# monkey0head/RePlay_cql

Measured on NVIDIA B200. Metric: CQL updates/sec (batch 1024), higher is better.
Workload: dtype f32 (f16x3: tensor-core fp16 hi/lo 3-term split with exact power-of-two row scales, fp32 accumulate, 1e-4 parity-gated)

## Files before the change

### replay_cql_b200/csrc/capi.cu

```cuda
#include <cstring>
#include <cstdio>
#include <algorithm>
#include "engine.cuh"
#include "update.cuh"
#include "score.cuh"
#include "tc_selftest.cuh"
#include "score_tc.cuh"
#include "score_tc_h.cuh"
#include "topk_staged.cuh"
#include "metrics.cuh"
#include "dp_peer.cuh"
#include "mma_bench.cuh"

using namespace cql;

struct cql_handle {
  Handle h;
  cudaGraphExec_t graph_exec = nullptr;
  cudaStream_t graph_stream = nullptr;
  int64_t graph_launches = 0;
  cudaGraphExec_t batch_graph[2] = {nullptr, nullptr};
  cudaStream_t batch_graph_stream[2] = {nullptr, nullptr};
  int64_t batch_graph_launches[2] = {0, 0};
  void* sbuf[8] = {nullptr, nullptr, nullptr, nullptr, nullptr, nullptr, nullptr, nullptr};
// ... 19 lines not shown
};

static thread_local std::string g_create_error;

int64_t mdp_build_on_device(Handle& h, const int32_t* user_h, const int32_t* item_h, const int64_t* ts_h, const double* rel_h,
                            const double* noise_h, int64_t n, int top_k, float noise_scale, float* obs_out, float* act_out,
                            float* rew_out, float* term_out, int64_t* order_out);

namespace {

void* scratch(cql_handle* ch, int slot, size_t bytes) {
  if (bytes > ch->sbuf_bytes[slot]) {
    if (ch->sbuf[slot]) CQL_CUDA(cudaFree(ch->sbuf[slot]));
    ch->sbuf[slot] = nullptr;
    ch->sbuf_bytes[slot] = 0;
    const size_t cap = bytes + bytes / 4 + 256;
    CQL_CUDA(cudaMalloc(&ch->sbuf[slot], cap));
    ch->sbuf_bytes[slot] = cap;
  }
  return ch->sbuf[slot];
}

void set_kernel_attrs() {
  CQL_CUDA(cudaFuncSetAttribute(mlp_fwd_kernel<2, 2>, cudaFuncAttributeMaxDynamicSharedMemorySize, FWD_SMEM));
  CQL_CUDA(cudaFuncSetAttribute(mlp_fwd_kernel<3, 1>, cudaFuncAttributeMaxDynamicSharedMemorySize, FWD_SMEM));
  CQL_CUDA(cudaFuncSetAttribute(mlp_bwd1_kernel<3, 1, true, false>, cudaFuncAttributeMaxDynamicSharedMemorySize, BWD1_SMEM));
  CQL_CUDA(cudaFuncSetAttribute(mlp_bwd1_kernel<3, 1, false, true>, cudaFuncAttributeMaxDynamicSharedMemorySize, BWD1_SMEM));
  CQL_CUDA(cudaFuncSetAttribute(mlp_bwd1_kernel<2, 2, true, false>, cudaFuncAttributeMaxDynamicSharedMemorySize, BWD1_SMEM));
  CQL_CUDA(cudaFuncSetAttribute(mlp_bwd2_kernel<3, 1>, cudaFuncAttributeMaxDynamicSharedMemorySize, BWD2_SMEM));
  CQL_CUDA(cudaFuncSetAttribute(mlp_bwd2_kernel<2, 2>, cudaFuncAttributeMaxDynamicSharedMemorySize, BWD2_SMEM));
  CQL_CUDA(cudaFuncSetAttribute(k_score_topk, cudaFuncAttributeMaxDynamicSharedMemorySize, score_smem(CQL_MAX_TOPK)));
  CQL_CUDA(cudaFuncSetAttribute(k_score_pairs, cudaFuncAttributeMaxDynamicSharedMemorySize, FWD_SMEM));
  CQL_CUDA(cudaFuncSetAttribute(k_topk_filter_staged, cudaFuncAttributeMaxDynamicSharedMemorySize, (int)TKS_SMEM));
  CQL_CUDA(cudaFuncSetAttribute(tc::tc_fwd_kernel<true, 2, 2>, cudaFuncAttributeMaxDynamicSharedMemorySize, (int)tc::FwdSmem<true, tc::FWD_NPW>::BYTES));
  CQL_CUDA(cudaFuncSetAttribute(tc::tc_fwd_kernel<true, 3, 1>, cudaFuncAttributeMaxDynamicSharedMemorySize, (int)tc::FwdSmem<true, tc::FWD_NPW>::BYTES));
  CQL_CUDA(cudaFuncSetAttribute(tc::tc_fwd_kernel<false, 2, 2>, cudaFuncAttributeMaxDynamicSharedMemorySize, (int)tc::FwdSmem<false, tc::FWD_NPW>::BYTES));
  CQL_CUDA(cudaFuncSetAttribute(tc::tc_fwd_kernel<false, 3, 1>, cudaFuncAttributeMaxDynamicSharedMemorySize, (int)tc::FwdSmem<false, tc::FWD_NPW>::BYTES));
  CQL_CUDA(cudaFuncSetAttribute(tc::tc_score_kernel, cudaFuncAttributeMaxDynamicSharedMemorySize, (int)tc::ScoreSmem::bytes(CQL_MAX_TOPK)));
  CQL_CUDA(cudaFuncSetAttribute(tc::tc_score_h_kernel, cudaFuncAttributeMaxDynamicSharedMemorySize, (int)tc::ScoreSmemH::bytes(CQL_MAX_TOPK)));
  CQL_CUDA(cudaFuncSetAttribute(tc::tc_bwd2_h_kernel<3, 1>, cudaFuncAttributeMaxDynamicSharedMemorySize, (int)tc::B2HCfg::BYTES));
  CQL_CUDA(cudaFuncSetAttribute(tc::tc_bwd2_h_kernel<2, 2>, cudaFuncAttributeMaxDynamicSharedMemorySize, (int)tc::B2HCfg::BYTES));
  CQL_CUDA(cudaFuncSetAttribute(tc::tc_bwd2_h2_kernel<3, 1>, cudaFuncAttributeMaxDynamicSharedMemorySize, (int)tc::B2PCfg::BYTES));
  CQL_CUDA(cudaFuncSetAttribute(tc::tc_bwd2_h2_kernel<2, 2>, cudaFuncAttributeMaxDynamicSharedMemorySize, (int)tc::B2PCfg::BYTES));
  CQL_CUDA(cudaFuncSetAttribute(tc::tc_bwd1_h_kernel<3, 1, true, false>, cudaFuncAttributeMaxDynamicSharedMemorySize, (int)tc::HCfg::SMEM_BYTES));
  CQL_CUDA(cudaFuncSetAttribute(tc::tc_bwd1_h_kernel<3, 1, false, true>, cudaFuncAttributeMaxDynamicSharedMemorySize, (int)tc::HCfg::SMEM_BYTES));
  CQL_CUDA(cudaFuncSetAttribute(tc::tc_bwd1_h_kernel<2, 2, true, false>, cudaFuncAttributeMaxDynamicSharedMemorySize, (int)tc::HCfg::SMEM_BYTES));
  CQL_CUDA(cudaFuncSetAttribute(tc::tc_fwd_h_kernel<2, 2>, cudaFuncAttributeMaxDynamicSharedMemorySize, (int)tc::HCfg::SMEM_BYTES));
  CQL_CUDA(cudaFuncSetAttribute(tc::tc_fwd_h_kernel<3, 1>, cudaFuncAttributeMaxDynamicSharedMemorySize, (int)tc::HCfg::SMEM_BYTES));
  CQL_CUDA(cudaFuncSetAttribute((tc::tc_fwd_h_kernel<3, 1, tc::HCfgS>), cudaFuncAttributeMaxDynamicSharedMemorySize, (int)tc::HCfgS::SMEM_BYTES));
  CQL_CUDA(cudaFuncSetAttribute((tc::tc_fwd_h_kernel<2, 2, tc::HCfgS>), cudaFuncAttributeMaxDynamicSharedMemorySize, (int)tc::HCfgS::SMEM_BYTES));
  CQL_CUDA(cudaFuncSetAttribute((tc::tc_bwd1_h_kernel<3, 1, true, false, tc::HCfgS>), cudaFuncAttributeMaxDynamicSharedMemorySize, (int)tc::HCfgS::SMEM_BYTES));
  CQL_CUDA(cudaFuncSetAttribute((tc::tc_bwd1_h_kernel<3, 1, false, true, tc::HCfgS>), cudaFuncAttributeMaxDynamicSharedMemorySize, (int)tc::HCfgS::SMEM_BYTES));
  CQL_CUDA(cudaFuncSetAttribute((tc::tc_bwd1_h_kernel<2, 2, true, false, tc::HCfgS>), cudaFuncAttributeMaxDynamicSharedMemorySize, (int)tc::HCfgS::SMEM_BYTES));
  CQL_CUDA(cudaFuncSetAttribute(tc::tc_fwd_h2_kernel<3, 1>, cudaFuncAttributeMaxDynamicSharedMemorySize, (int)tc::H2Cfg::SMEM_BYTES));
  CQL_CUDA(cudaFuncSetAttribute(tc::tc_fwd_h2_kernel<2, 2>, cudaFuncAttributeMaxDynamicSharedMemorySize, (int)tc::H2Cfg::SMEM_BYTES));
  CQL_CUDA(cudaFuncSetAttribute(tc::tc_bwd1_h2_kernel<3, 1, true, false>, cudaFuncAttributeMaxDynamicSharedMemorySize, (int)tc::H2B1Cfg::SMEM_BYTES));
  CQL_CUDA(cudaFuncSetAttribute(tc::tc_bwd1_h2_kernel<3, 1, false, true>, cudaFuncAttributeMaxDynamicSharedMemorySize, (int)tc::H2B1Cfg::SMEM_BYTES));
  CQL_CUDA(cudaFuncSetAttribute(tc::tc_bwd1_h2_kernel<2, 2, true, false>, cudaFuncAttributeMaxDynamicSharedMemorySize, (int)tc::H2B1Cfg::SMEM_BYTES));
  CQL_CUDA(cudaFuncSetAttribute(tc::tc_fwd_ts_kernel<2, 2>, cudaFuncAttributeMaxDynamicSharedMemorySize, (int)tc::TsCfg::SMEM_BYTES));
  CQL_CUDA(cudaFuncSetAttribute(tc::tc_fwd_ts_kernel<3, 1>, cudaFuncAttributeMaxDynamicSharedMemorySize, (int)tc::TsCfg::SMEM_BYTES));
  CQL_CUDA(cudaFuncSetAttribute(tc::tc_bwd1_ts_kernel<3, 1, true, false>, cudaFuncAttributeMaxDynamicSharedMemorySize, (int)tc::TsCfg::SMEM_BYTES));
  CQL_CUDA(cudaFuncSetAttribute(tc::tc_bwd1_ts_kernel<3, 1, false, true>, cudaFuncAttributeMaxDynamicSharedMemorySize, (int)tc::TsCfg::SMEM_BYTES));
  CQL_CUDA(cudaFuncSetAttribute(tc::tc_bwd1_ts_kernel<2, 2, true, false>, cudaFuncAttributeMaxDynamicSharedMemorySize, (int)tc::TsCfg::SMEM_BYTES));
  const int f1 = (int)tc::FwdSmem<true, tc::BWD1_NPW>::BYTES, f0 = (int)tc::FwdSmem<false, tc::BWD1_NPW>::BYTES;
  CQL_CUDA(cudaFuncSetAttribute(tc::tc_bwd1_kernel<true, 3, 1, true, false>, cudaFuncAttributeMaxDynamicSharedMemorySize, f1));
  CQL_CUDA(cudaFuncSetAttribute(tc::tc_bwd1_kernel<true, 3, 1, false, true>, cudaFuncAttributeMaxDynamicSharedMemorySize, f1));
  CQL_CUDA(cudaFuncSetAttribute(tc::tc_bwd1_kernel<true, 2, 2, true, false>, cudaFuncAttributeMaxDynamicSharedMemorySize, f1));
  CQL_CUDA(cudaFuncSetAttribute(tc::tc_bwd1_kernel<false, 3, 1, true, false>, cudaFuncAttributeMaxDynamicSharedMemorySize, f0));
  CQL_CUDA(cudaFuncSetAttribute(tc::tc_bwd1_kernel<false, 3, 1, false, true>, cudaFuncAttributeMaxDynamicSharedMemorySize, f0));
  CQL_CUDA(cudaFuncSetAttribute(tc::tc_bwd1_kernel<false, 2, 2, true, false>, cudaFuncAttributeMaxDynamicSharedMemorySize, f0));
  CQL_CUDA(cudaFuncSetAttribute(tc::tc_bwd2_kernel<true, 3, 1>, cudaFuncAttributeMaxDynamicSharedMemorySize, (int)tc::B2Cfg<true>::BYTES));
  CQL_CUDA(cudaFuncSetAttribute(tc::tc_bwd2_kernel<true, 2, 2>, cudaFuncAttributeMaxDynamicSharedMemorySize, (int)tc::B2Cfg<true>::BYTES));
  CQL_CUDA(cudaFuncSetAttribute(tc::tc_bwd2_kernel<false, 3, 1>, cudaFuncAttributeMaxDynamicSharedMemorySize, (int)tc::B2Cfg<false>::BYTES));
  CQL_CUDA(cudaFuncSetAttribute(tc::tc_bwd2_kernel<false, 2, 2>, cudaFuncAttributeMaxDynamicSharedMemorySize, (int)tc::B2Cfg<false>::BYTES));
}

void create_impl(const cql_config* cfg, cql_handle* ch) {
  Handle& h = ch->h;
  CQL_REQUIRE(cfg != nullptr, "cql_create: cfg is NULL");
  CQL_REQUIRE(cfg->struct_size == (int32_t)sizeof(cql_config), "cql_create: cql_config size mismatch (ABI)");
  CQL_REQUIRE(cfg->batch_size >= 1 && cfg->batch_size <= (1 << 20), "cql_create: batch_size out of range");
  CQL_REQUIRE(cfg->n_critics >= 1 && cfg->n_critics <= CQL_MAX_CRITICS, "cql_create: n_critics must be 1..4");
  CQL_REQUIRE(cfg->n_action_samples >= 1 && cfg->n_action_samples <= 10, "cql_create: n_action_samples must be 1..10");
  CQL_REQUIRE(cfg->precision == CQL_PREC_FP32 || cfg->precision == CQL_PREC_TF32X3 || cfg->precision == CQL_PREC_BF16 ||
                  cfg->precision == CQL_PREC_F16X3,
              "cql_create: bad precision");
  CQL_REQUIRE(cfg->squash == CQL_SQUASH_EPS || cfg->squash == CQL_SQUASH_SOFTPLUS, "cql_create: bad squash");
  CQL_REQUIRE(cfg->world_size >= 1 && cfg->rank >= 0 && cfg->rank < cfg->world_size, "cql_create: bad rank/world_size");
  int ndev = 0;
  cudaError_t e = cudaGetDeviceCount(&ndev);
  if (e != cudaSuccess || ndev == 0)
    throw Error{std::string("cql_create: no CUDA device available (") + cudaGetErrorString(e) +
                "); this library has no CPU fallback"};
  CQL_REQUIRE(cfg->device >= 0 && cfg->device < ndev, "cql_create: device ordinal out of range");
  CQL_CUDA(cudaSetDevice(cfg->device));
  cudaDeviceProp prop{};
  CQL_CUDA(cudaGetDeviceProperties(&prop, cfg->device));
  CQL_REQUIRE(prop.major >= 10, "cql_create: built for sm_100a (B200); found an older GPU");
  h.cfg = *cfg;
  h.num_sms = prop.multiProcessorCount;
  h.B = cfg->batch_size; h.n = cfg->n_action_samples; h.C = cfg->n_critics;
  const int B = h.B, n = h.n, C = h.C, n3 = 3 * n;
  h.rsA = n3; h.rsC = n3 + 1;
  CQL_CUDA(cudaStreamCreateWithFlags(&h.own_stream, cudaStreamNonBlocking));
  CQL_CUDA(cudaStreamCreateWithFlags(&h.side_stream, cudaStreamNonBlocking));
  CQL_CUDA(cudaEventCreateWithFlags(&h.ev_fork, cudaEventDisableTiming));
// ... 952 lines not shown
```

### replay_cql_b200/csrc/update.cuh

```cuda
#pragma once
#include <algorithm>
#include <utility>
#include <cstdlib>
#include "engine.cuh"
#include "mlp_tc.cuh"
#include "mlp_tc_ts.cuh"
#include <type_traits>
#include "mlp_tc_bwd1.cuh"
#include "mlp_tc_bwd2.cuh"
#include "mlp_tc_h.cuh"
#include "mlp_tc_h2.cuh"
#include "adam_pack.cuh"

namespace cql {

__host__ __device__ inline uint32_t mix32(uint32_t x) {
  x ^= x >> 16; x *= 0x7feb352du; x ^= x >> 15; x *= 0x846ca68bu; x ^= x >> 16;
  return x;
}
__host__ __device__ inline uint64_t feistel_perm(uint64_t x, uint64_t n, uint64_t key) {
  int bits = 2;
  while (bits < 62 && (1ull << bits) < n) bits += 2;
  const int hb = bits / 2;
  const uint64_t mask = (1ull << hb) - 1;
// ... 417 lines not shown
    __shared__ float gsh[2];
    if (threadIdx.x == 0) dp_wait_scalars(dp, g_t, g_a, gsh[0], gsh[1]);
    __syncthreads();
    g_t = gsh[0];
    g_a = gsh[1];
  }
  if (k.temp_lr > 0.f) lt = adam_scalar(lt, g_t, mt, vt, k.temp_lr, k, *si);
  if (k.alpha_lr > 0.f) la = adam_scalar(la, g_a, ma, va, k.alpha_lr, k, *si);
  const float alpha = fminf(fmaxf(expf(la), 0.f), 1e6f);
  const float inv = 1.f / ((float)k.C * (float)k.B);
  const float coef = alpha * k.cw * inv;
  const int64_t i = (int64_t)blockIdx.x * blockDim.x + threadIdx.x;
  const int rsC = 3 * k.n + 1;
  if (i < (int64_t)k.C * k.B * rsC) {
    const int j = (int)(i % rsC);
    dQ[i] = j < rsC - 1 ? coef * dQ[i] : 2.f * pairv[i / rsC].err / (float)k.B - coef;
  }
  if (i == 0) {
    if (k.temp_lr > 0.f) { scalars[0] = lt; sc_m[0] = mt; sc_v[0] = vt; }
    if (k.alpha_lr > 0.f) { scalars[1] = la; sc_m[1] = ma; sc_v[1] = va; }
    sums[3] = coef;
    metrics[1] = expf(lt);
    metrics[3] = expf(la);
    const float td = sums[0] / (float)k.B;
    const float cons = alpha * (k.cw * (sums[1] * inv - sums[2] * inv) - k.thr);
    metrics[4] = td + cons;
    metrics[6] = td;
  }
  if (dp.world > 1) dp_consume_done(dp, 0, gridDim.x);
}

__global__ void __launch_bounds__(1024) k_actor_dq(const QSrc srcP, const float4* __restrict__ perb,
                                                   const float* __restrict__ scalars, int B, int C,
                                                   float* __restrict__ dQP, float* __restrict__ metrics) {
  tc::grid_dep_wait();
 
  __shared__ float red[32];
  const float T = expf(scalars[0]);
  float s = 0.f;
  for (int b = threadIdx.x; b < B; b += 1024) {
    int arg = 0;
    float qm = q_at(srcP, 0, b);
    for (int c = 1; c < C; ++c) {
      const float q = q_at(srcP, c, b);
      if (q < qm) { qm = q; arg = c; }
    }
    for (int c = 0; c < C; ++c) dQP[(int64_t)c * B + b] = c == arg ? -1.f / (float)B : 0.f;
    s += T * perb[b].y - qm;
  }
  s = block_sum<1024>(s, red);
  if (threadIdx.x == 0) metrics[5] = s / (float)B;
}

__global__ void k_actor_dout(const float* __restrict__ outA, const float* __restrict__ noise_actor,
                             const float4* __restrict__ dXP, const float* __restrict__ scalars, int B, int n_parts,
                             int squash, float* __restrict__ dOutA, const QSrc srcP, const float4* __restrict__ perb,
                             int C, float* __restrict__ part, unsigned int* __restrict__ ticket, float* __restrict__ metrics) {
  tc::grid_dep_wait();
 
  const int b = blockIdx.x * blockDim.x + threadIdx.x;
  if (srcP.q != nullptr) {
    float v = 0.f;
    if (b < B) {
      float qm = q_at(srcP, 0, b);
      for (int c = 1; c < C; ++c) qm = fminf(qm, q_at(srcP, c, b));
      v = expf(scalars[0]) * perb[b].y - qm;
    }
    v = warp_sum(v);
    if ((threadIdx.x & 31) == 0) part[b >> 5] = v;
    __shared__ bool last;
    __threadfence();
    __syncthreads();
    if (threadIdx.x == 0) {
      const unsigned int t = atomicAdd(ticket, 1u);
      last = t == gridDim.x - 1;
      if (last) *ticket = 0;
    }
    __syncthreads();
    if (last && threadIdx.x < 32) {
      __threadfence();
      const int n_w = (gridDim.x * blockDim.x) >> 5;
      float s = 0.f;
      for (int i = threadIdx.x; i < n_w; i += 32) s += part[i];
      s = warp_sum(s);
      if (threadIdx.x == 0) metrics[5] = s / (float)B;
    }
  }
  if (b >= B) return;
  float da = 0.f;
  for (int c = 0; c < n_parts; ++c) da += dXP[(int64_t)c * B + b].z;
  const float mu = outA[2 * b], ls_raw = outA[2 * b + 1], ls = clamp_ls(ls_raw);
  const float eps = noise_actor[b];
  const Sample s = policy_sample(mu, ls, eps, squash);
  const float w = __fdiv_rn(expf(scalars[0]), (float)B);
  const float one_m_a2 = __fsub_rn(1.f, __fmul_rn(s.a, s.a));
  const float dt_std = __fmul_rn(w, __fdiv_rn(s.t, s.std_));
  float g_tanh;
  if (squash == CQL_SQUASH_EPS) {
    const float g_a = __fadd_rn(da, __fmul_rn(w, __fdiv_rn(__fmul_rn(2.f, s.a), __fadd_rn(one_m_a2, 1e-6f))));
    g_tanh = __fmul_rn(g_a, one_m_a2);
  } else {
    const float sig = __fdiv_rn(1.f, __fadd_rn(1.f, expf(__fmul_rn(2.f, s.raw))));
    g_tanh = __fadd_rn(__fmul_rn(w, __fsub_rn(2.f, __fmul_rn(4.f, sig))), __fmul_rn(da, one_m_a2));
  }
  const float g_raw = __fadd_rn(g_tanh, -dt_std);
  const float g_mu = __fadd_rn(g_raw, dt_std);
  const float g_std = __fadd_rn(__fmul_rn(g_raw, eps), __fmul_rn(w, __fdiv_rn(__fmul_rn(s.t, s.t), s.std_)));
  const float g_ls = __fsub_rn(__fmul_rn(g_std, s.std_), w);
  dOutA[2 * b] = g_mu;
  dOutA[2 * b + 1] = (ls_raw >= -20.f && ls_raw <= 2.f) ? g_ls : 0.f;
}

__global__ void k_reduce_grads(const float* __restrict__ small, const float* __restrict__ pw2, int in_dim, int out_dim,
                               int tiles, int splits, float* __restrict__ grads) {
  const int net = blockIdx.y;
  const int idx = blockIdx.x * blockDim.x + threadIdx.x;
  if (idx >= NET_STRIDE) return;
  const int w2_lo = off_W2(in_dim), w2_hi = w2_lo + H * H, total = net_floats(in_dim, out_dim);
  float s = 0.f;
  if (idx >= w2_lo && idx < w2_hi) {
    const float* p = pw2 + (size_t)net * splits * H * H + (idx - w2_lo);
    for (int i = 0; i < splits; ++i) s += p[(size_t)i * H * H];
  } else if (idx < total) {
    const int sidx = idx < w2_lo ? idx : idx - H * H;
    const float* p = small + (size_t)net * tiles * SMALL_STRIDE + sidx;
    for (int i = 0; i < tiles; ++i) s += p[(size_t)i * SMALL_STRIDE];
  }
  grads[(size_t)net * NET_STRIDE + idx] = s;
}

__global__ void k_adam_polyak(float* __restrict__ p, float* __restrict__ m, float* __restrict__ v,
                              const float* __restrict__ g, float* __restrict__ targ, int64_t count, float lr,
                              float beta1, float beta2, float eps, float tau, const StepInfo* __restrict__ si) {
  tc::grid_dep_wait();
 
  const int64_t i = (int64_t)blockIdx.x * blockDim.x + threadIdx.x;
  if (i >= count) return;
  const float step_size = (float)((double)lr / si->bc1);
  const float bc2s = (float)si->bc2_sqrt;
  const float gi = g[i];
  const float mi = m[i] + (gi - m[i]) * (1.f - beta1);
  const float vi = v[i] * beta2 + (1.f - beta2) * gi * gi;
  m[i] = mi;
  v[i] = vi;
  const float pn = p[i] - step_size * (mi / (sqrtf(vi) / bc2s + eps));
  p[i] = pn;
  if (targ) targ[i] = targ[i] * (1.f - tau) + tau * pn;
}

inline bool g_timing_no_pdl = false;
inline bool skip_launch(int bit) {
  static const int mask = std::getenv("CQL_SKIP") ? std::atoi(std::getenv("CQL_SKIP")) : 0;
  return (mask & bit) != 0;
}
template <typename... KArgs, typename... Args>
inline void launch_pdl(void (*kernel)(KArgs...), dim3 grid, dim3 block, size_t smem, cudaStream_t st, Args&&... args) {
  static const bool no_pdl_env = std::getenv("CQL_NO_PDL") != nullptr;
  const bool no_pdl = no_pdl_env || g_timing_no_pdl;
  cudaLaunchConfig_t cfg{};
  cfg.gridDim = grid; cfg.blockDim = block; cfg.dynamicSmemBytes = smem; cfg.stream = st;
  cudaLaunchAttribute attr[1];
  attr[0].id = cudaLaunchAttributeProgrammaticStreamSerialization;
  attr[0].val.programmaticStreamSerializationAllowed = 1;
  cfg.attrs = attr;
// ... 364 lines not shown
  }
  CQL_LAUNCH_CHECK(h);
  {
    FwdJobs jobs{};
    jobs.n = 3;
    jobs.j[0] = FwdJob{h->XAl, h->net_params(slot_critic(0)), h->QAl, nullptr, B * n3, C, 0};
    jobs.j[1] = FwdJob{h->XC, h->net_params(slot_critic(0)), h->QC, h->h2C, B * (n3 + 1), C, 0};
    jobs.j[2] = FwdJob{h->XT, h->net_params(slot_targ_critic(C, 0)), h->QT, nullptr, B, C, 0};
    mark(h, st, 3);
    QSrc srcQ[3];
    for (int rep = 0; rep < (h->timing ? TIMED_FWD_REPS : 1); ++rep) {
      const bool saved = g_timing_no_pdl;
      if (rep > 0) g_timing_no_pdl = false;
      launch_fwd_any<3, 1>(h, jobs, st, srcQ);
      g_timing_no_pdl = saved;
    }
    mark(h, st, 4);
    const int64_t so = scalars_off(C);
    ScalarReduceArgs ra{reinterpret_cast<const float4*>(h->perb), h->scalars(), h->adam_m + so, h->adam_v + so, h->g_scalars(),
                        h->loss_sums, h->metrics, reinterpret_cast<unsigned int*>(h->loss_sums + 15), h->dp_fused ? h->dp : DpPeer{}};
    if (!skip_launch(2))
      launch_pdl(k_lse, dim3((C * B * 32 + 255) / 256), dim3(256), 0, st, batch4, srcQ[0], h->offAl, srcQ[1], h->offC, srcQ[2], loss_consts(h),
               h->dQ, reinterpret_cast<PairVals*>(h->pairv), ra);
    CQL_LAUNCH_CHECK(h);
  }
}

inline void phase1(Handle* h, cudaStream_t st) {
  NvtxRange nvtx("cql.update.phase1: temp/alpha Adam, critic backward");
  const int B = h->B, C = h->C, n3 = 3 * h->n, rows = B * (n3 + 1);
  const int64_t so = scalars_off(C);
  if (!skip_launch(8))
    launch_pdl(k_scalar_adam_dq, dim3((int)(((int64_t)C * rows + 255) / 256)), dim3(256), 0, st, h->scalars(), h->adam_m + so, h->adam_v + so,
             h->g_scalars(), h->stepinfo, loss_consts(h), h->loss_sums, h->metrics, reinterpret_cast<const PairVals*>(h->pairv), h->dQ,
             h->dp_fused ? h->dp : DpPeer{}, (long long)(1 + C) * NET_STRIDE);
  CQL_LAUNCH_CHECK(h);
  BwdJob jb{h->XC, h->dQ, h->h2C, h->net_params(slot_critic(0)), h->smallC, nullptr, h->pw2C, rows, C, h->splitsC};
  mark(h, st, 5);
  if (h->cfg.precision != CQL_PREC_FP32) {
    if (h->cfg.precision == CQL_PREC_F16X3) launch_bwd_tc<true, 3, 1, true, false, true>(h, jb, h->g_critics(), st, 6, 7);
    else if (h->cfg.precision != CQL_PREC_BF16) launch_bwd_tc<true, 3, 1, true, false>(h, jb, h->g_critics(), st, 6, 7);
    else launch_bwd_tc<false, 3, 1, true, false>(h, jb, h->g_critics(), st, 6, 7);
    return;
  }
  launch_bwd1<3, 1, true, false>(h, jb, st);
  mark(h, st, 6);
  launch_bwd2<3, 1>(h, jb, st);
  mark(h, st, 7);
  k_reduce_grads<<<dim3((NET_STRIDE + 255) / 256, C), 256, 0, st>>>(h->smallC, h->pw2C, 3, 1, tiles_of(rows),
                                                                   h->splitsC, h->g_critics());
  CQL_LAUNCH_CHECK(h);
}

inline void phase2(Handle* h, cudaStream_t st) {
  NvtxRange nvtx("cql.update.phase2: critic Adam + Polyak + pack, actor step forward/backward");
  const int B = h->B, C = h->C;
  const cql_config& c = h->cfg;
  static const bool no_fused_adam = std::getenv("CQL_NO_FUSED_ADAM") != nullptr;
  if (h->cfg.precision == CQL_PREC_F16X3 && !no_fused_adam) {
    adam_pack(h, slot_critic(0), C, 3, 1, c.critic_lr, st);
  } else {
    const int64_t cnt = (int64_t)C * NET_STRIDE;
    launch_pdl(k_adam_polyak, dim3((int)((cnt + 255) / 256)), dim3(256), 0, st,
        h->net_params(slot_critic(0)), h->adam_m + (size_t)NET_STRIDE, h->adam_v + (size_t)NET_STRIDE, h->g_critics(),
        h->net_params(slot_targ_critic(C, 0)), cnt, c.critic_lr, c.beta1, c.beta2, c.adam_eps, c.tau, h->stepinfo);
    CQL_LAUNCH_CHECK(h);
    int slots[2 * CQL_MAX_CRITICS];
    for (int i = 0; i < C; ++i) { slots[i] = slot_critic(i); slots[C + i] = slot_targ_critic(C, i); }
    pack_slots(h, slots, 2 * C, st);
  }
  bool fold_dq = false;
  QSrc srcP_keep{};
  {
    FwdJobs jobs{};
    jobs.n = 1;
    jobs.j[0] = FwdJob{h->XP, h->net_params(slot_critic(0)), h->QP, h->h2P, B, C, 0};
    mark(h, st, 8);
    QSrc srcP[1];
    launch_fwd_any<3, 1>(h, jobs, st, srcP);
    mark(h, st, 9);
    fold_dq = h->cfg.precision == CQL_PREC_F16X3 && srcP[0].n_parts > 0;
    srcP_keep = srcP[0];
    if (!fold_dq) {
      if (!skip_launch(16))
        launch_pdl(k_actor_dq, dim3(1), dim3(1024), 0, st, srcP[0], reinterpret_cast<const float4*>(h->perb), h->scalars(), B, C, h->dQP,
                 h->metrics);
      CQL_LAUNCH_CHECK(h);
    }
  }
  {
    BwdJob jb{h->XP, h->dQP, h->h2P, h->net_params(slot_critic(0)), nullptr, h->dXP, nullptr, B, C, 1};
    if (fold_dq) { jb.q_part = srcP_keep.q; jb.q_parts = srcP_keep.n_parts; jb.dq_scale = -1.f / (float)B; }
    if (h->cfg.precision == CQL_PREC_F16X3) launch_bwd_tc<true, 3, 1, false, true, true>(h, jb, nullptr, st);
    else if (h->cfg.precision == CQL_PREC_TF32X3) launch_bwd_tc<true, 3, 1, false, true>(h, jb, nullptr, st);
    else if (h->cfg.precision == CQL_PREC_BF16) launch_bwd_tc<false, 3, 1, false, true>(h, jb, nullptr, st);
    else launch_bwd1<3, 1, false, true>(h, jb, st);
  }
  const bool tcm = h->cfg.precision != CQL_PREC_FP32;
  if (!skip_launch(32))
    launch_pdl(k_actor_dout, dim3((B + 127) / 128), dim3(128), 0, st, h->outA, h->noise + B + 6 * (int64_t)B * h->n,
                                                tcm ? h->dX_part : h->dXP, h->scalars(), B,
                                                tcm ? h->last_dx_parts : C, c.squash, h->dOutA,
                                                fold_dq ? srcP_keep : QSrc{}, reinterpret_cast<const float4*>(h->perb), C,
                                                h->actor_part, reinterpret_cast<unsigned int*>(h->loss_sums + 14), h->metrics);
  CQL_LAUNCH_CHECK(h);
  BwdJob ja{h->XA, h->dOutA, h->h2A, h->net_params(slot_actor()), h->smallA, nullptr, h->pw2A, B, 1, h->splitsA};
  mark(h, st, 10);
  if (tcm) {
    if (h->cfg.precision == CQL_PREC_F16X3) launch_bwd_tc<true, 2, 2, true, false, true>(h, ja, h->g_actor(), st);
    else if (h->cfg.precision != CQL_PREC_BF16) launch_bwd_tc<true, 2, 2, true, false>(h, ja, h->g_actor(), st);
    else launch_bwd_tc<false, 2, 2, true, false>(h, ja, h->g_actor(), st);
    mark(h, st, 11);
    return;
  }
  launch_bwd1<2, 2, true, false>(h, ja, st);
  launch_bwd2<2, 2>(h, ja, st);
  mark(h, st, 11);
  k_reduce_grads<<<dim3((NET_STRIDE + 255) / 256, 1), 256, 0, st>>>(h->smallA, h->pw2A, 2, 2, tiles_of(B), h->splitsA,
                                                                   h->g_actor());
  CQL_LAUNCH_CHECK(h);
}

inline void phase3(Handle* h, cudaStream_t st) {
  NvtxRange nvtx("cql.update.phase3: actor Adam + Polyak + pack");
  const cql_config& c = h->cfg;
  static const bool no_fused_adam = std::getenv("CQL_NO_FUSED_ADAM") != nullptr;
  if (h->cfg.precision == CQL_PREC_F16X3 && !no_fused_adam) {
    adam_pack(h, slot_actor(), 1, 2, 2, c.actor_lr, st, true);
    mark(h, st, 12);
    return;
  } else {
    launch_pdl(k_adam_polyak, dim3((NET_STRIDE + 255) / 256), dim3(256), 0, st, h->net_params(slot_actor()), h->adam_m, h->adam_v,
                                                           h->g_actor(), h->net_params(slot_targ_actor(h->C)),
                                                           (int64_t)NET_STRIDE, c.actor_lr, c.beta1, c.beta2, c.adam_eps,
                                                           c.tau, h->stepinfo);
    CQL_LAUNCH_CHECK(h);
    pack_weights(h, slot_actor(), 1, 2, st);
  }
  launch_pdl(k_step_end, dim3(1), dim3(1), 0, st, h->step_dev);
  CQL_LAUNCH_CHECK(h);
  mark(h, st, 12);
}

}
```

Before: 4637.

## Fuse actor-step critic forward, dQ, backward and dout into one cluster kernel

Adds a thread-block-cluster kernel that, for small batches and up to two critics, runs the critic forward, the min-Q argmin gradient, the critic input backward and the actor output gradient in a single launch. Partial Q values, ReLU sign masks and dX partials are exchanged through distributed shared memory with cluster mbarriers. This replaces the separate forward, dQ, backward and dout launches and their global round-trips. The cost is a complex synchronisation scheme, and the fused path is gated on having enough SMs for the work.

```diff
diff --git a/replay_cql_b200/csrc/actor_step_h.cuh b/replay_cql_b200/csrc/actor_step_h.cuh
--- /dev/null
+++ b/replay_cql_b200/csrc/actor_step_h.cuh
@@ -0,0 +1,364 @@
+#pragma once
+#include "mlp_tc_h2.cuh"
+
+namespace cql {
+namespace tc {
+
+struct ActorStepJob {
+  const float4* X;
+  const float* params;
+  const uint8_t* packed;
+  const uint8_t* packedT;
+  const float* outA;
+  const float* noise_actor;
+  const float* scalars;
+  const float4* perb;
+  float* dOutA;
+  float* part;
+  unsigned int* ticket;
+  float* metrics;
+  int rows, n_nets, squash;
+};
+
+struct ASCfg {
+  using C = HCfgT<8, 64>;
+  static constexpr int SLICES = C::SLICES;
+  static constexpr int MAXC = 2;
+  static constexpr int PARTS = HCfgS::SLICES;
+  static constexpr uint32_t OFF_B = 0;
+  static constexpr uint32_t OFF_W1 = 2 * C::B_BYTES;
+  static constexpr uint32_t OFF_W3 = OFF_W1 + H * 16;
+  static constexpr uint32_t OFF_EB = OFF_W3 + H * 4;
+  static constexpr uint32_t OFF_IV = OFF_EB + 2 * C::NS * 16;
+  static constexpr uint32_t OFF_Q = OFF_IV + C::NS * 4;
+  static constexpr uint32_t OFF_SIGN = OFF_Q + MAXC * PARTS * TM * 4;
+  static constexpr uint32_t OFF_DX = OFF_SIGN + MAXC * PARTS * TM * 4;
+  static constexpr uint32_t OFF_BAR = OFF_DX + MAXC * PARTS * TM * 4;
+  static constexpr uint32_t N_BARS = 2 * C::STAGES + 2 + 2 + 2;
+  static constexpr uint32_t OFF_SLOT = OFF_BAR + N_BARS * 8;
+  static constexpr uint32_t SMEM_BYTES = OFF_SLOT + 16;
+};
+static_assert(ASCfg::SMEM_BYTES <= 227 * 1024, "actor-step kernel: shared memory");
+static_assert(ASCfg::MAXC * ASCfg::SLICES <= 8, "actor-step kernel: portable cluster size");
+
+__device__ __forceinline__ uint32_t cluster_nctarank() {
+  uint32_t r;
+  asm volatile("mov.u32 %0, %%cluster_nctarank;" : "=r"(r));
+  return r;
+}
+__device__ __forceinline__ uint32_t cluster_addr(const void* p, uint32_t cta) {
+  uint32_t r;
+  asm volatile("mapa.shared::cluster.u32 %0, %1, %2;" : "=r"(r) : "r"(smem_u32(p)), "r"(cta));
+  return r;
+}
+__device__ __forceinline__ void st_cluster(uint32_t addr, float v) {
+  asm volatile("st.shared::cluster.f32 [%0], %1;" ::"r"(addr), "f"(v) : "memory");
+}
+__device__ __forceinline__ void st_cluster(uint32_t addr, uint32_t v) {
+  asm volatile("st.shared::cluster.u32 [%0], %1;" ::"r"(addr), "r"(v) : "memory");
+}
+__device__ __forceinline__ void fence_cluster() { asm volatile("fence.acq_rel.cluster;" ::: "memory"); }
+__device__ __forceinline__ void mbar_arrive_release_cluster(uint32_t bar_addr) {
+  asm volatile("mbarrier.arrive.release.cluster.shared::cluster.b64 _, [%0];" ::"r"(bar_addr) : "memory");
+}
+__device__ __forceinline__ void mbar_wait_acquire_cluster(uint64_t* bar, uint32_t parity) {
+  uint32_t ok;
+  do {
+    asm volatile(
+        "{\n\t.reg .pred p;\n\tmbarrier.try_wait.parity.acquire.cluster.shared::cta.b64 p, [%1], %2;\n\t"
+        "selp.u32 %0, 1, 0, p;\n\t}"
+        : "=r"(ok)
+        : "r"(smem_u32(bar)), "r"(parity)
+        : "memory");
+  } while (!ok);
+}
+
+__global__ void __launch_bounds__(HCfgS::THREADS, 1) tc_actor_critic_h_kernel(const ActorStepJob jb) {
+  using A = ASCfg;
+  using C = A::C;
+  constexpr int IN = 3;
+  extern __shared__ __align__(1024) uint8_t sm[];
+  uint8_t* Bs = sm + A::OFF_B;
+  float4* w1p = reinterpret_cast<float4*>(sm + A::OFF_W1);
+  float* w3s = reinterpret_cast<float*>(sm + A::OFF_W3);
+  float4* ebs = reinterpret_cast<float4*>(sm + A::OFF_EB);
+  float* ivg = reinterpret_cast<float*>(sm + A::OFF_IV);
+  float* qs = reinterpret_cast<float*>(sm + A::OFF_Q);
+  uint32_t* signs = reinterpret_cast<uint32_t*>(sm + A::OFF_SIGN);
+  float* dxs = reinterpret_cast<float*>(sm + A::OFF_DX);
+  uint64_t* bars = reinterpret_cast<uint64_t*>(sm + A::OFF_BAR);
+  uint64_t* full = bars;
+  uint64_t* empty = bars + C::STAGES;
+  uint64_t* tfull = bars + 2 * C::STAGES;
+  uint64_t* bload = tfull + 2;
+  uint64_t* qready = bload + 2;
+  uint64_t* dxready = qready + 1;
+  uint32_t* slot = reinterpret_cast<uint32_t*>(sm + A::OFF_SLOT);
+
+  const int tid = threadIdx.x, warp = tid >> 5, lane = tid & 31;
+  const uint32_t rank = cluster_ctarank(), n_ranks = cluster_nctarank();
+  const int net_i = (int)rank / A::SLICES, slice = (int)rank % A::SLICES, tile = blockIdx.x / (int)n_ranks;
+  const int n = jb.n_nets;
+  const float* net = jb.params + (size_t)net_i * NET_STRIDE;
+  const uint8_t* opF = jb.packed + (size_t)net_i * HCfg::PACKED_NET_BYTES;
+  const uint8_t* opB = jb.packedT + (size_t)net_i * HCfg::PACKED_NET_BYTES;
+  const HMeta* metaF = reinterpret_cast<const HMeta*>(opF + HCfg::META_OFF);
+  const HMeta* metaB = reinterpret_cast<const HMeta*>(opB + HCfg::META_OFF);
+  auto load_b3 = [&]() {
+    return make_float2(__ldg(jb.params + off_b3(IN, 1)), n > 1 ? __ldg(jb.params + NET_STRIDE + off_b3(IN, 1)) : 0.f);
+  };
+  auto q_of = [&](int c, int rt, float2 b3) {
+    const float bias = c == 0 ? b3.x : b3.y;
+    float v = 0.f;
+#pragma unroll
+    for (int p = 0; p < A::PARTS; ++p) v += qs[(c * A::PARTS + p) * TM + rt];
+    return v + bias;
+  };
+  auto dq_of = [&](int rt, float2 b3) {
+    int arg = 0;
+    float qm = 0.f;
+    for (int c = 0; c < n; ++c) {
+      const float q = q_of(c, rt, b3);
+      if (c == 0 || q < qm) { qm = q; arg = c; }
+    }
+    return net_i == arg ? -1.f / (float)jb.rows : 0.f;
+  };
+
+  if (warp == C::MMA_WARP) {
+    tmem_alloc(slot, C::TMEM_ALLOC);
+    if (lane == 0) {
+      for (int s = 0; s < C::STAGES; ++s) { mbar_init(&full[s], C::NPW); mbar_init(&empty[s], 1); }
+      for (int a = 0; a < 2; ++a) { mbar_init(&tfull[a], 1); mbar_init(&bload[a], 1); }
+      mbar_init(qready, n_ranks * 128);
+      mbar_init(dxready, n_ranks * 128);
+      fence_mbar_init();
+    }
+  }
+  tc_fence_before();
+  __syncthreads();
+  tc_fence_after();
+  cluster_sync_all();
+  const uint32_t tmem = *slot;
+  grid_dep_wait();
+
+  if (warp == C::MMA_WARP) {
+    const uint32_t idesc = instr_desc(FMT_F16, TM, C::NS);
+    const uint32_t b_lbo = C::NS * 16;
+    if (elect_one()) {
+      load_operand_slice<C>(Bs, opF, slice, &bload[0]);
+      load_operand_slice<C>(Bs + C::B_BYTES, opB, slice, &bload[1]);
+    }
+    __syncwarp();
+    uint32_t it = 0;
+    for (int i = 0; i < 2; ++i) {
+      mbar_wait(&bload[i], 0);
+      const uint32_t b_base = smem_u32(Bs + i * C::B_BYTES);
+      const uint32_t d_tmem = tmem + i * C::NS;
+      tc_fence_after();
+      for (int c = 0; c < C::NCHUNK; ++c, ++it) {
+        const uint32_t s = it % C::STAGES;
+        mbar_wait(&full[s], (it / C::STAGES) & 1);
+        tc_fence_after();
+        if (elect_one()) {
+          const uint32_t a_stage = tmem + C::A_COL0 + s * C::A_STAGE_COLS;
+#pragma unroll
+          for (int j = 0; j < C::KC / C::UK; ++j) {
+            const uint32_t g = c * (C::KC / C::UK) + j;
+            const uint64_t b_hi = smem_desc(b_base + 2 * g * b_lbo, b_lbo, 128);
+            const uint64_t b_lo = smem_desc(b_base + C::B_TERM_BYTES + 2 * g * b_lbo, b_lbo, 128);
+            const uint32_t a_hi = a_stage + j * 8, a_lo = a_hi + C::A_LO_COLS;
+            umma_ts<false>(d_tmem, a_lo, b_hi, idesc, (c == 0 && j == 0) ? 0u : 1u);
+            umma_ts<false>(d_tmem, a_hi, b_lo, idesc, 1u);
+            umma_ts<false>(d_tmem, a_hi, b_hi, idesc, 1u);
+          }
+          umma_commit(&empty[s]);
+          if (c == C::NCHUNK - 1) umma_commit(&tfull[i]);
+        }
+        __syncwarp();
+      }
+    }
+  } else if (warp >= C::NEW) {
+    const int pw = warp - C::NEW, ptid = tid - C::NEW * 32;
+    const int kq = pw >> 2;
+    const uint32_t lane_base = tmem + ((uint32_t)((warp & 3) * 32) << 16) + C::A_COL0 + kq * (C::KPW / 2);
+    const int rt = (warp & 3) * 32 + lane, r = tile * TM + rt;
+    const bool ok = r < jb.rows;
+    const float4 x = ok ? __ldg(jb.X + r) : make_float4(0.f, 0.f, 0.f, 0.f);
+    for (int pr = ptid; pr < H / 2; pr += C::PROD_THREADS) {
+      const int k = 2 * pr;
+      const float* wa = net + off_W1(IN) + k * IN;
+      const float* wb = wa + IN;
+      w1p[2 * pr] = make_float4(wa[0], wb[0], wa[1], wb[1]);
+      w1p[2 * pr + 1] = make_float4(wa[2], wb[2], net[off_b1(IN) + k], net[off_b1(IN) + k + 1]);
+      w3s[k] = net[off_W3(IN) + k];
+      w3s[k + 1] = net[off_W3(IN) + k + 1];
+    }
+    asm volatile("bar.sync 1, %0;" ::"n"(C::PROD_THREADS));
+    uint32_t it = 0;
+    {
+      const float4 wm = make_float4(__ldg(&metaF->wmax[0]), __ldg(&metaF->wmax[1]), __ldg(&metaF->wmax[2]), __ldg(&metaF->wmax[3]));
+      float sa, inv_sa;
+      pow2_scale(h1_row_bound(x, wm), sa, inv_sa);
+      const float2 xx = make_float2(x.x, x.x), xy = make_float2(x.y, x.y), xz = make_float2(x.z, x.z), ss = make_float2(sa, sa);
+      for (int c = 0; c < C::NCHUNK; ++c, ++it) {
+        const uint32_t s = it % C::STAGES;
+        uint32_t hi[C::KPW / 2], lo[C::KPW / 2];
+#pragma unroll
+        for (int pp = 0; pp < C::KPW / 2; ++pp) {
+          const int pr = (c * C::KC + kq * C::KPW) / 2 + pp;
+          const float4 wA = w1p[2 * pr], wB = w1p[2 * pr + 1];
+          float2 v = ffma2(xx, make_float2(wA.x, wA.y), make_float2(wB.z, wB.w));
+          v = ffma2(xy, make_float2(wA.z, wA.w), v);
+          v = ffma2(xz, make_float2(wB.x, wB.y), v);
+          v = fmul2(make_float2(fmaxf(v.x, 0.f), fmaxf(v.y, 0.f)), ss);
+          split_h2_trunc(v, hi[pp], lo[pp]);
+        }
+        mbar_wait(&empty[s], ((it / C::STAGES) & 1) ^ 1);
+        tc_fence_after();
+        tmem_st8(lane_base + s * C::A_STAGE_COLS, hi);
+        tmem_st8(lane_base + s * C::A_STAGE_COLS + C::A_LO_COLS, lo);
+        tmem_st_wait();
+        tc_fence_before();
+        __syncwarp();
+        if (lane == 0) mbar_arrive(&full[s]);
+      }
+    }
+    {
+      const float w3m0 = __ldg(&metaB->wmax[4]);
+      const float2 b3 = load_b3();
+      mbar_wait_acquire_cluster(qready, 0);
+      const float d0 = ok ? dq_of(rt, b3) : 0.f;
+      float sa, inv_sa;
+      pow2_scale(fmaf(fabsf(d0), w3m0, 0.f), sa, inv_sa);
+      const float d0s = d0 * sa;
+      for (int c = 0; c < C::NCHUNK; ++c, ++it) {
+        const uint32_t s = it % C::STAGES;
+        const int j0 = c * C::KC + kq * C::KPW;
+        const uint32_t sg = signs[(net_i * A::PARTS + (j0 >> 5)) * TM + rt] >> (j0 & 31);
+        uint32_t hi[C::KPW / 2], lo[C::KPW / 2];
+#pragma unroll
+        for (int e = 0; e < C::KPW; e += 2) {
+          const float ga = d0s * w3s[j0 + e], gb = d0s * w3s[j0 + e + 1];
+          split_h2_trunc(make_float2((sg >> e) & 1u ? ga : 0.f, (sg >> (e + 1)) & 1u ? gb : 0.f), hi[e / 2], lo[e / 2]);
+        }
+        mbar_wait(&empty[s], ((it / C::STAGES) & 1) ^ 1);
+        tc_fence_after();
+        tmem_st8(lane_base + s * C::A_STAGE_COLS, hi);
+        tmem_st8(lane_base + s * C::A_STAGE_COLS + C::A_LO_COLS, lo);
+        tmem_st_wait();
+        tc_fence_before();
+        __syncwarp();
+        if (lane == 0) mbar_arrive(&full[s]);
+      }
+    }
+  } else {
+    const int grp = warp >> 2, qw = warp & 3, gtid = tid & 127;
+    float4* ebg = ebs + grp * C::NS;
+    const int rt = qw * 32 + lane, row = tile * TM + rt;
+    const bool ok = row < jb.rows;
+    const int k = slice * C::NS + gtid;
+    const uint32_t tm_row = tmem + ((uint32_t)(qw * 32) << 16) + grp * C::NS;
+    if (grp == 0) {
+      if (gtid < C::NS) ebg[gtid] = make_float4(net[off_b2(IN) + k], net[off_W3(IN) + k], 0.f, __ldg(&metaF->inv_s[k]));
+      const float4 wm = make_float4(__ldg(&metaF->wmax[0]), __ldg(&metaF->wmax[1]), __ldg(&metaF->wmax[2]), __ldg(&metaF->wmax[3]));
+      const float4 x = ok ? __ldg(jb.X + row) : make_float4(0.f, 0.f, 0.f, 0.f);
+      asm volatile("bar.sync 2, 128;");
+      float sa, inv_sa;
+      pow2_scale(h1_row_bound(x, wm), sa, inv_sa);
+      mbar_wait(&tfull[0], 0);
+      tc_fence_after();
+      float q0[2];
+      uint32_t sg[2];
+#pragma unroll 1
+      for (int h = 0; h < 2; ++h) {
+        float v[32];
+        tmem_ld32(tm_row + h * 32, v);
+        tmem_ld_wait();
+        q0[h] = 0.f;
+        sg[h] = 0;
+#pragma unroll
+        for (int j = 0; j < 32; ++j) {
+          const float4 e = ebg[h * 32 + j];
+          const float hv = fmaxf(fmaf(v[j] * inv_sa, e.w, e.x), 0.f);
+          q0[h] = fmaf(hv, e.y, q0[h]);
+          sg[h] |= (hv > 0.f ? 1u : 0u) << j;
+        }
+      }
+      const int at = (net_i * A::PARTS + slice * 2) * TM + rt;
+      for (uint32_t p = 0; p < n_ranks; ++p) {
+        st_cluster(cluster_addr(qs + at, p), q0[0]);
+        st_cluster(cluster_addr(qs + at + TM, p), q0[1]);
+        st_cluster(cluster_addr(signs + at, p), sg[0]);
+        st_cluster(cluster_addr(signs + at + TM, p), sg[1]);
+      }
+      fence_cluster();
+      for (uint32_t p = 0; p < n_ranks; ++p) mbar_arrive_release_cluster(cluster_addr(qready, p));
+    } else {
+      if (gtid < C::NS) {
+        ebg[gtid] = make_float4(net[off_W1(IN) + k * IN], net[off_W1(IN) + k * IN + 1], net[off_W1(IN) + k * IN + 2], net[off_b1(IN) + k]);
+        ivg[gtid] = __ldg(&metaB->inv_s[k]);
+      }
+      const float w3m0 = __ldg(&metaB->wmax[4]);
+      const float4 x = ok ? __ldg(jb.X + row) : make_float4(0.f, 0.f, 0.f, 0.f);
+      const float2 b3 = load_b3();
+      asm volatile("bar.sync 3, 128;");
+      mbar_wait_acquire_cluster(qready, 0);
+      const float d0 = ok ? dq_of(rt, b3) : 0.f;
+      float sa, inv_sa;
+      pow2_scale(fmaf(fabsf(d0), w3m0, 0.f), sa, inv_sa);
+      mbar_wait(&tfull[1], 0);
+      tc_fence_after();
+      float dx2[2];
+#pragma unroll 1
+      for (int h = 0; h < 2; ++h) {
+        float v[32];
+        tmem_ld32(tm_row + h * 32, v);
+        tmem_ld_wait();
+        dx2[h] = 0.f;
+#pragma unroll
+        for (int j = 0; j < 32; ++j) {
+          const float4 w = ebg[h * 32 + j];
+          float z = fmaf(x.y, w.y, fmaf(x.x, w.x, w.w));
+          z = fmaf(x.z, w.z, z);
+          const float d = z > 0.f ? v[j] * inv_sa * ivg[h * 32 + j] : 0.f;
+          dx2[h] = fmaf(d, w.z, dx2[h]);
+        }
+      }
+      const int at = (net_i * A::PARTS + slice * 2) * TM + rt;
+      st_cluster(cluster_addr(dxs + at, 0), dx2[0]);
+      st_cluster(cluster_addr(dxs + at + TM, 0), dx2[1]);
+      fence_cluster();
+      mbar_arrive_release_cluster(cluster_addr(dxready, 0));
+    }
+  }
+  tc_fence_before();
+  __syncthreads();
+  if (warp == C::MMA_WARP) tmem_dealloc(tmem, C::TMEM_ALLOC);
+  if (rank == 0) {
+    const int b = tile * TM + tid;
+    const bool mine = tid < TM && b < jb.rows;
+    const float log_temp = jb.scalars[0];
+    const float lp = mine ? jb.perb[b].y : 0.f;
+    const float mu = mine ? jb.outA[2 * b] : 0.f, ls_raw = mine ? jb.outA[2 * b + 1] : 0.f;
+    const float eps = mine ? jb.noise_actor[b] : 0.f;
+    const float2 b3 = load_b3();
+    float v = 0.f;
+    if (tid < TM) mbar_wait_acquire_cluster(dxready, 0);
+    if (mine) {
+      float qm = q_of(0, tid, b3);
+      for (int c = 1; c < n; ++c) qm = fminf(qm, q_of(c, tid, b3));
+      v = expf(log_temp) * lp - qm;
+    }
+    actor_loss_metric(v, tid < TM ? b >> 5 : -1, (int)(gridDim.x / n_ranks) * (TM / 32), jb.rows, jb.part, jb.ticket,
+                      gridDim.x / n_ranks, jb.metrics);
+    if (mine) {
+      float da = 0.f;
+      for (int p = 0; p < n * A::PARTS; ++p) da += dxs[p * TM + tid];
+      actor_dout_row(mu, ls_raw, eps, log_temp, jb.rows, jb.squash, b, da, jb.dOutA);
+    }
+  }
+  cluster_sync_all();
+}
+
+}
+}
diff --git a/replay_cql_b200/csrc/capi.cu b/replay_cql_b200/csrc/capi.cu
--- a/replay_cql_b200/csrc/capi.cu
+++ b/replay_cql_b200/csrc/capi.cu
@@ -95,6 +95,7 @@
   CQL_CUDA(cudaFuncSetAttribute((tc::tc_bwd1_h_kernel<3, 1, true, false, tc::HCfgS>), cudaFuncAttributeMaxDynamicSharedMemorySize, (int)tc::HCfgS::SMEM_BYTES));
   CQL_CUDA(cudaFuncSetAttribute((tc::tc_bwd1_h_kernel<3, 1, false, true, tc::HCfgS>), cudaFuncAttributeMaxDynamicSharedMemorySize, (int)tc::HCfgS::SMEM_BYTES));
   CQL_CUDA(cudaFuncSetAttribute((tc::tc_bwd1_h_kernel<2, 2, true, false, tc::HCfgS>), cudaFuncAttributeMaxDynamicSharedMemorySize, (int)tc::HCfgS::SMEM_BYTES));
+  CQL_CUDA(cudaFuncSetAttribute(tc::tc_actor_critic_h_kernel, cudaFuncAttributeMaxDynamicSharedMemorySize, (int)tc::ASCfg::SMEM_BYTES));
   CQL_CUDA(cudaFuncSetAttribute(tc::tc_fwd_h2_kernel<3, 1>, cudaFuncAttributeMaxDynamicSharedMemorySize, (int)tc::H2Cfg::SMEM_BYTES));
   CQL_CUDA(cudaFuncSetAttribute(tc::tc_fwd_h2_kernel<2, 2>, cudaFuncAttributeMaxDynamicSharedMemorySize, (int)tc::H2Cfg::SMEM_BYTES));
   CQL_CUDA(cudaFuncSetAttribute(tc::tc_bwd1_h2_kernel<3, 1, true, false>, cudaFuncAttributeMaxDynamicSharedMemorySize, (int)tc::H2B1Cfg::SMEM_BYTES));
diff --git a/replay_cql_b200/csrc/update.cuh b/replay_cql_b200/csrc/update.cuh
--- a/replay_cql_b200/csrc/update.cuh
+++ b/replay_cql_b200/csrc/update.cuh
@@ -493,6 +493,52 @@
   if (threadIdx.x == 0) metrics[5] = s / (float)B;
 }
 
+__device__ __forceinline__ void actor_loss_metric(float v, int slot, int n_slots, int B, float* __restrict__ part,
+                                                  unsigned int* __restrict__ ticket, unsigned int n_blocks,
+                                                  float* __restrict__ metrics) {
+  v = warp_sum(v);
+  if ((threadIdx.x & 31) == 0 && slot >= 0) part[slot] = v;
+  __shared__ bool last;
+  __threadfence();
+  __syncthreads();
+  if (threadIdx.x == 0) {
+    const unsigned int t = atomicAdd(ticket, 1u);
+    last = t == n_blocks - 1;
+    if (last) *ticket = 0;
+  }
+  __syncthreads();
+  if (last && threadIdx.x < 32) {
+    __threadfence();
+    float s = 0.f;
+    for (int i = threadIdx.x; i < n_slots; i += 32) s += part[i];
+    s = warp_sum(s);
+    if (threadIdx.x == 0) metrics[5] = s / (float)B;
+  }
+}
+
+__device__ __forceinline__ void actor_dout_row(float mu, float ls_raw, float eps, float log_temp, int B, int squash, int b,
+                                               float da, float* __restrict__ dOutA) {
+  const float ls = clamp_ls(ls_raw);
+  const Sample s = policy_sample(mu, ls, eps, squash);
+  const float w = __fdiv_rn(expf(log_temp), (float)B);
+  const float one_m_a2 = __fsub_rn(1.f, __fmul_rn(s.a, s.a));
+  const float dt_std = __fmul_rn(w, __fdiv_rn(s.t, s.std_));
+  float g_tanh;
+  if (squash == CQL_SQUASH_EPS) {
+    const float g_a = __fadd_rn(da, __fmul_rn(w, __fdiv_rn(__fmul_rn(2.f, s.a), __fadd_rn(one_m_a2, 1e-6f))));
+    g_tanh = __fmul_rn(g_a, one_m_a2);
+  } else {
+    const float sig = __fdiv_rn(1.f, __fadd_rn(1.f, expf(__fmul_rn(2.f, s.raw))));
+    g_tanh = __fadd_rn(__fmul_rn(w, __fsub_rn(2.f, __fmul_rn(4.f, sig))), __fmul_rn(da, one_m_a2));
+  }
+  const float g_raw = __fadd_rn(g_tanh, -dt_std);
+  const float g_mu = __fadd_rn(g_raw, dt_std);
+  const float g_std = __fadd_rn(__fmul_rn(g_raw, eps), __fmul_rn(w, __fdiv_rn(__fmul_rn(s.t, s.t), s.std_)));
+  const float g_ls = __fsub_rn(__fmul_rn(g_std, s.std_), w);
+  dOutA[2 * b] = g_mu;
+  dOutA[2 * b + 1] = (ls_raw >= -20.f && ls_raw <= 2.f) ? g_ls : 0.f;
+}
+
 __global__ void k_actor_dout(const float* __restrict__ outA, const float* __restrict__ noise_actor,
                              const float4* __restrict__ dXP, const float* __restrict__ scalars, int B, int n_parts,
                              int squash, float* __restrict__ dOutA, const QSrc srcP, const float4* __restrict__ perb,
@@ -507,50 +553,17 @@
       for (int c = 1; c < C; ++c) qm = fminf(qm, q_at(srcP, c, b));
       v = expf(scalars[0]) * perb[b].y - qm;
     }
-    v = warp_sum(v);
-    if ((threadIdx.x & 31) == 0) part[b >> 5] = v;
-    __shared__ bool last;
-    __threadfence();
-    __syncthreads();
-    if (threadIdx.x == 0) {
-      const unsigned int t = atomicAdd(ticket, 1u);
-      last = t == gridDim.x - 1;
-      if (last) *ticket = 0;
-    }
-    __syncthreads();
-    if (last && threadIdx.x < 32) {
-      __threadfence();
-      const int n_w = (gridDim.x * blockDim.x) >> 5;
-      float s = 0.f;
-      for (int i = threadIdx.x; i < n_w; i += 32) s += part[i];
-      s = warp_sum(s);
-      if (threadIdx.x == 0) metrics[5] = s / (float)B;
-    }
+    actor_loss_metric(v, b >> 5, (gridDim.x * blockDim.x) >> 5, B, part, ticket, gridDim.x, metrics);
   }
   if (b >= B) return;
   float da = 0.f;
   for (int c = 0; c < n_parts; ++c) da += dXP[(int64_t)c * B + b].z;
-  const float mu = outA[2 * b], ls_raw = outA[2 * b + 1], ls = clamp_ls(ls_raw);
-  const float eps = noise_actor[b];
-  const Sample s = policy_sample(mu, ls, eps, squash);
-  const float w = __fdiv_rn(expf(scalars[0]), (float)B);
-  const float one_m_a2 = __fsub_rn(1.f, __fmul_rn(s.a, s.a));
-  const float dt_std = __fmul_rn(w, __fdiv_rn(s.t, s.std_));
-  float g_tanh;
-  if (squash == CQL_SQUASH_EPS) {
-    const float g_a = __fadd_rn(da, __fmul_rn(w, __fdiv_rn(__fmul_rn(2.f, s.a), __fadd_rn(one_m_a2, 1e-6f))));
-    g_tanh = __fmul_rn(g_a, one_m_a2);
-  } else {
-    const float sig = __fdiv_rn(1.f, __fadd_rn(1.f, expf(__fmul_rn(2.f, s.raw))));
-    g_tanh = __fadd_rn(__fmul_rn(w, __fsub_rn(2.f, __fmul_rn(4.f, sig))), __fmul_rn(da, one_m_a2));
-  }
-  const float g_raw = __fadd_rn(g_tanh, -dt_std);
-  const float g_mu = __fadd_rn(g_raw, dt_std);
-  const float g_std = __fadd_rn(__fmul_rn(g_raw, eps), __fmul_rn(w, __fdiv_rn(__fmul_rn(s.t, s.t), s.std_)));
-  const float g_ls = __fsub_rn(__fmul_rn(g_std, s.std_), w);
-  dOutA[2 * b] = g_mu;
-  dOutA[2 * b + 1] = (ls_raw >= -20.f && ls_raw <= 2.f) ? g_ls : 0.f;
-}
+  actor_dout_row(outA[2 * b], outA[2 * b + 1], noise_actor[b], scalars[0], B, squash, b, da, dOutA);
+}
+
+}
+#include "actor_step_h.cuh"
+namespace cql {
 
 __global__ void k_reduce_grads(const float* __restrict__ small, const float* __restrict__ pw2, int in_dim, int out_dim,
                                int tiles, int splits, float* __restrict__ grads) {
@@ -1021,23 +1034,9 @@
   CQL_LAUNCH_CHECK(h);
 }
 
-inline void phase2(Handle* h, cudaStream_t st) {
-  NvtxRange nvtx("cql.update.phase2: critic Adam + Polyak + pack, actor step forward/backward");
+inline void actor_step_critic_pass(Handle* h, cudaStream_t st) {
   const int B = h->B, C = h->C;
   const cql_config& c = h->cfg;
-  static const bool no_fused_adam = std::getenv("CQL_NO_FUSED_ADAM") != nullptr;
-  if (h->cfg.precision == CQL_PREC_F16X3 && !no_fused_adam) {
-    adam_pack(h, slot_critic(0), C, 3, 1, c.critic_lr, st);
-  } else {
-    const int64_t cnt = (int64_t)C * NET_STRIDE;
-    launch_pdl(k_adam_polyak, dim3((int)((cnt + 255) / 256)), dim3(256), 0, st,
-        h->net_params(slot_critic(0)), h->adam_m + (size_t)NET_STRIDE, h->adam_v + (size_t)NET_STRIDE, h->g_critics(),
-        h->net_params(slot_targ_critic(C, 0)), cnt, c.critic_lr, c.beta1, c.beta2, c.adam_eps, c.tau, h->stepinfo);
-    CQL_LAUNCH_CHECK(h);
-    int slots[2 * CQL_MAX_CRITICS];
-    for (int i = 0; i < C; ++i) { slots[i] = slot_critic(i); slots[C + i] = slot_targ_critic(C, i); }
-    pack_slots(h, slots, 2 * C, st);
-  }
   bool fold_dq = false;
   QSrc srcP_keep{};
   {
@@ -1073,9 +1072,60 @@
                                                 fold_dq ? srcP_keep : QSrc{}, reinterpret_cast<const float4*>(h->perb), C,
                                                 h->actor_part, reinterpret_cast<unsigned int*>(h->loss_sums + 14), h->metrics);
   CQL_LAUNCH_CHECK(h);
+}
+
+inline bool actor_step_fusable(const Handle* h) {
+  static const bool no_fused_actor = std::getenv("CQL_NO_FUSED_ACTOR") != nullptr;
+  static const bool no_small = std::getenv("CQL_NO_SMALL") != nullptr;
+  const int items128 = h->C * tc::HCfg::SLICES * ((h->B + tc::TM - 1) / tc::TM);
+  return !no_fused_actor && !no_small && h->C <= tc::ASCfg::MAXC && items128 * 2 <= h->num_sms;
+}
+
+inline void phase2(Handle* h, cudaStream_t st) {
+  NvtxRange nvtx("cql.update.phase2: critic Adam + Polyak + pack, actor step forward/backward");
+  const int B = h->B, C = h->C;
+  const cql_config& c = h->cfg;
+  static const bool no_fused_adam = std::getenv("CQL_NO_FUSED_ADAM") != nullptr;
+  if (h->cfg.precision == CQL_PREC_F16X3 && !no_fused_adam) {
+    adam_pack(h, slot_critic(0), C, 3, 1, c.critic_lr, st);
+  } else {
+    const int64_t cnt = (int64_t)C * NET_STRIDE;
+    launch_pdl(k_adam_polyak, dim3((int)((cnt + 255) / 256)), dim3(256), 0, st,
+        h->net_params(slot_critic(0)), h->adam_m + (size_t)NET_STRIDE, h->adam_v + (size_t)NET_STRIDE, h->g_critics(),
+        h->net_params(slot_targ_critic(C, 0)), cnt, c.critic_lr, c.beta1, c.beta2, c.adam_eps, c.tau, h->stepinfo);
+    CQL_LAUNCH_CHECK(h);
+    int slots[2 * CQL_MAX_CRITICS];
+    for (int i = 0; i < C; ++i) { slots[i] = slot_critic(i); slots[C + i] = slot_targ_critic(C, i); }
+    pack_slots(h, slots, 2 * C, st);
+  }
+  if (h->cfg.precision == CQL_PREC_F16X3 && actor_step_fusable(h)) {
+    mark(h, st, 8);
+    const tc::ActorStepJob j{h->XP, h->net_params(slot_critic(0)),
+                             h->packed_fwd + (size_t)slot_critic(0) * h->packed_net_bytes,
+                             h->packed_bwd + (size_t)slot_critic(0) * h->packed_net_bytes_bwd,
+                             h->outA, h->noise + B + 6 * (int64_t)B * h->n, h->scalars(), reinterpret_cast<const float4*>(h->perb),
+                             h->dOutA, h->actor_part, reinterpret_cast<unsigned int*>(h->loss_sums + 14), h->metrics, B, C, c.squash};
+    const int ranks = tc::ASCfg::SLICES * C;
+    cudaLaunchConfig_t cfg{};
+    cfg.gridDim = dim3(ranks * ((B + tc::TM - 1) / tc::TM)); cfg.blockDim = dim3(tc::HCfgS::THREADS);
+    cfg.dynamicSmemBytes = tc::ASCfg::SMEM_BYTES; cfg.stream = st;
+    cudaLaunchAttribute attr[2];
+    attr[0].id = cudaLaunchAttributeClusterDimension;
+    attr[0].val.clusterDim.x = ranks; attr[0].val.clusterDim.y = 1; attr[0].val.clusterDim.z = 1;
+    attr[1].id = cudaLaunchAttributeProgrammaticStreamSerialization;
+    attr[1].val.programmaticStreamSerializationAllowed = 1;
+    static const bool no_pdl_env = std::getenv("CQL_NO_PDL") != nullptr;
+    cfg.attrs = attr;
+    cfg.numAttrs = (no_pdl_env || g_timing_no_pdl) ? 1 : 2;
+    CQL_CUDA(cudaLaunchKernelEx(&cfg, tc::tc_actor_critic_h_kernel, j));
+    CQL_LAUNCH_CHECK(h);
+    mark(h, st, 9);
+  } else {
+    actor_step_critic_pass(h, st);
+  }
   BwdJob ja{h->XA, h->dOutA, h->h2A, h->net_params(slot_actor()), h->smallA, nullptr, h->pw2A, B, 1, h->splitsA};
   mark(h, st, 10);
-  if (tcm) {
+  if (h->cfg.precision != CQL_PREC_FP32) {
     if (h->cfg.precision == CQL_PREC_F16X3) launch_bwd_tc<true, 2, 2, true, false, true>(h, ja, h->g_actor(), st);
     else if (h->cfg.precision != CQL_PREC_BF16) launch_bwd_tc<true, 2, 2, true, false>(h, ja, h->g_actor(), st);
     else launch_bwd_tc<false, 2, 2, true, false>(h, ja, h->g_actor(), st);
```

Result: faster. 4703, median of 6 (+1.4%).
